# jrcalgo/RelayRL-prototype

Hardware: AMD Instinct MI355X
Metric: env steps/sec (whole node) + wall-clock to return threshold, CartPole REINFORCE (higher is better)
Workload: dtype fp32; 1 GPU; global_batch=2097152, seq_len=64, parallelism=dp1, envs_per_gpu=32768, train_vf_iters=80, hyperparams=reference defaults (gamma .98, lam .97, pi_lr 3e-4, vf_lr 1e-3)

## Files before the change

### csrc/kernels/value_grad.hip

```cpp
#include "common.h"
#include "grad_args.h"
#include "heads.h"

namespace rrl {

typedef __bf16 vbf16x8 __attribute__((ext_vector_type(8)));
typedef __bf16 vbf16x4 __attribute__((ext_vector_type(4)));
typedef short vs16x4 __attribute__((ext_vector_type(4)));

constexpr int kVgH = 128;
#ifndef VG_MT2
#define VG_MT2 1
#endif
constexpr int kVgLd = 144;
constexpr int kVgImg = 64 * kVgLd;
constexpr int vg_red_bytes(int NA) { return 8 * 64 * NA * 4; }
constexpr int vg_base_bytes(int DP, int NA) {
  return 6 * kVgImg * 2 + 2 * 64 * DP * 4 + (2 + NA) * 128 * 4 + 32 * 4 + kVgH * kVgLd * 2;
}
constexpr bool vg_red_in_image(int DP, int NA) { return vg_base_bytes(DP, NA) + vg_red_bytes(NA) > 160 * 1024; }
constexpr int vg_lds_bytes(int DP, int NA) {
  return vg_base_bytes(DP, NA) + (vg_red_in_image(DP, NA) ? 0 : vg_red_bytes(NA));
}
constexpr bool vg_factor(int DP, int HEAD, int NA) {
// ... 3 lines not shown
constexpr int vg_hbuf_bytes(int HEAD, int NA) {
  return HEAD == HEAD_VALUE_MSE ? 0 : 64 * 4 * (2 + ((HEAD == HEAD_PG_GAUSS || HEAD == HEAD_PPO_GAUSS) ? NA : 1));
}
constexpr bool vg_split_head(int HEAD, int NA) {
  return (HEAD == HEAD_PG_GAUSS || HEAD == HEAD_PPO_GAUSS) && NA > 1;
}
constexpr int vg_dtab_bytes(int HEAD, int NA) { return vg_split_head(HEAD, NA) ? (64 + 16) * NA * 4 : 0; }
constexpr int vg_dw_bytes(int DP, int HEAD, int NA) {
  return (vg_factor(DP, HEAD, NA) || (HEAD == HEAD_VALUE_MSE && vg_lds_bytes(DP, 1) + 8 * 64 * 4 <= 160 * 1024))
             ? 8 * 64 * 4
             : 0;
}
constexpr bool vg_hbuf2(int DP, int HEAD, int NA) {
  return !vg_red_in_image(DP, NA) && vg_lds_bytes(DP, NA) + vg_mask_bytes(DP, HEAD, NA) +
                                             2 * vg_hbuf_bytes(HEAD, NA) + vg_dtab_bytes(HEAD, NA) +
                                             vg_dw_bytes(DP, HEAD, NA) <=
                                         160 * 1024;
}
constexpr int vg_total_bytes(int DP, int HEAD, int NA) {
  return vg_lds_bytes(DP, NA) + vg_mask_bytes(DP, HEAD, NA) +
         (vg_red_in_image(DP, NA) ? 0 : (vg_hbuf2(DP, HEAD, NA) ? 2 : 1) * vg_hbuf_bytes(HEAD, NA)) +
         vg_dtab_bytes(HEAD, NA) + vg_dw_bytes(DP, HEAD, NA);
}
static_assert(vg_red_bytes(6) + vg_hbuf_bytes(HEAD_PPO_GAUSS, 6) <= 3 * kVgImg * 2, "head inputs in the dh2 image");
static_assert(vg_total_bytes(8, HEAD_VALUE_MSE, 1) <= 160 * 1024, "factored LDS plan");
static_assert(vg_total_bytes(4, HEAD_PG_CAT, 2) <= 160 * 1024 && vg_total_bytes(4, HEAD_PPO_CAT, 2) <= 160 * 1024,
              "factored binary policy LDS plan");
static_assert(vg_dw_bytes(20, HEAD_VALUE_MSE, 1) > 0 && vg_total_bytes(20, HEAD_VALUE_MSE, 1) <= 160 * 1024,
              "dout table of the D = 17..20 value kernel");
static_assert(vg_lds_bytes(24, 1) <= 160 * 1024 && !vg_red_in_image(24, 1), "value-grad LDS plan");
static_assert(vg_lds_bytes(20, 6) <= 160 * 1024, "value-grad LDS plan exceeds 160 KB");
static_assert(vg_red_bytes(6) <= 3 * kVgImg * 2, "head partials must fit in the dh2 image");

struct Split8 {
  vbf16x8 h, m, l;
};

struct Split8HM {
  vbf16x8 h, m;
};

typedef float vf32x2 __attribute__((ext_vector_type(2)));

RRL_DEV uint32_t cvt_pk_bf16(float a, float b) {
  typedef __bf16 vbf16x2_cvt __attribute__((ext_vector_type(2)));
  return __builtin_bit_cast(uint32_t, __builtin_convertvector((vf32x2{a, b}), vbf16x2_cvt));
// ... 163 lines not shown
  const bool hi = j & 1;
  const float send = hi ? w2[0] : w2[1], keep = hi ? w2[1] : w2[0];
  return keep + dpp_f<kDppXor1>(send);
}

RRL_DEV float wave_sum_vl(float v) {
  v += dpp_f<kDppXor1>(v);
  v += dpp_f<kDppXor2>(v);
  v += dpp_f<kDppMirror8>(v);
  v += dpp_f<kDppXor8>(v);
  return group_sum_swap(v);
}

#define VG_STAMP(k)                                                                     \
  if (STAMP) {                                                                          \
    __builtin_amdgcn_sched_barrier(0);                                                  \
    unsigned long long t_;                                                              \
    asm volatile("s_memtime %0\n\ts_waitcnt lgkmcnt(0)" : "=s"(t_)::"memory");          \
    __builtin_amdgcn_sched_barrier(0);                                                  \
    if ((k) > 0) st_sum[(k) > 0 ? (k)-1 : 0] += t_ - st_prev;                           \
    st_prev = t_;                                                                       \
  }

constexpr int vg_prod_v(int DP) { return DP <= 4 ? 3 : 1; }

template <int DP, int HEAD, int NA, bool STAMP = false, int V = vg_prod_v(DP), bool FWD = false>
__global__ __launch_bounds__(512, 1) void value_grad_split_kernel(GradArgs p) {
  unsigned long long st_prev = 0, st_sum[12] = {0, 0, 0, 0, 0, 0, 0, 0, 0, 0, 0, 0};
  unsigned long long st_entry = 0;
  if (STAMP) asm volatile("s_memtime %0\n\ts_waitcnt lgkmcnt(0)" : "=s"(st_entry)::"memory");
  extern __shared__ __attribute__((aligned(16))) uint16_t vg_lds[];
  constexpr bool kValue = HEAD == HEAD_VALUE_MSE;
  constexpr bool kGauss = HEAD == HEAD_PG_GAUSS || HEAD == HEAD_PPO_GAUSS;
  constexpr bool kPPO = HEAD == HEAD_PPO_CAT || HEAD == HEAD_PPO_GAUSS;
  static_assert(!kValue || NA == 1, "the value head has one output");
  static_assert(!FWD || kValue, "the forward-only instance is the value head's");
  static_assert(NA >= 1 && NA <= 6, "NA <= 6 (LDS plan, two field groups)");
  static_assert(!vg_split_head(HEAD, NA) || (NA % 2 == 0 && NA <= 6),
                "the dout table is read in output pairs; head MFMA lanes g = 0, 1 hold outputs 0..7");
  constexpr bool kFactor = vg_factor(DP, HEAD, NA) && !FWD;
  constexpr bool kBin = kFactor && !kValue;
  constexpr bool kMaskB = kFactor && (V & 1);
  constexpr bool kInterleave = kMaskB && (V & 2);
  constexpr int NF = NA + 2;
  constexpr int NG = (NF + 3) / 4;
  constexpr bool kRedImg = vg_red_in_image(DP, NA);
  constexpr bool kSplitHead = vg_split_head(HEAD, NA);
  uint16_t* h1img = vg_lds;
  uint16_t* dhimg = vg_lds + 3 * kVgImg;
  float* tail = reinterpret_cast<float*>(vg_lds + 6 * kVgImg);
  float* red = kRedImg ? reinterpret_cast<float*>(dhimg) : tail;
  float* xsb = kRedImg ? tail : tail + 8 * NA * 64;
  float* vecs = xsb + 2 * 64 * DP;
  uint16_t* w2lo = reinterpret_cast<uint16_t*>(vecs + (2 + NA) * kVgH + 32);
  uint32_t* mk = reinterpret_cast<uint32_t*>(w2lo + kVgH * kVgLd);
  const vbf16x8* mtab = reinterpret_cast<const vbf16x8*>(mk + 64 * 4);
  float* hbuf0 = kRedImg ? red + 8 * NA * 64
                         : reinterpret_cast<float*>(reinterpret_cast<char*>(mk) + vg_mask_bytes(DP, HEAD, NA));
  float* dtab = reinterpret_cast<float*>(
      reinterpret_cast<char*>(mk) + vg_mask_bytes(DP, HEAD, NA) +
      (kRedImg ? 0 : (vg_hbuf2(DP, HEAD, NA) ? 2 : 1) * vg_hbuf_bytes(HEAD, NA)));
  float* hacc = dtab + 64 * NA;
  if (kSplitHead && lane_id() < 2 * NA) hacc[(threadIdx.x >> 6) * 2 * NA + lane_id()] = 0.f;
  if (kMaskB) {
    for (int q = threadIdx.x; q < 256 * 4; q += blockDim.x) {
      const int i = q >> 2, e = 2 * (q & 3);
      mk[64 * 4 + q] = (((i >> e) & 1) ? 0x3F80u : 0u) | (((i >> (e + 1)) & 1) ? 0x3F800000u : 0u);
    }
  }
  int parity = 0;
  constexpr int KS1 = DP / 4;
  const int l = lane_id();
  const int j = l & 15, g = l >> 4, w = threadIdx.x >> 6;
  const int D = p.D;
  const int Bv = p.nvalid ? min(*p.nvalid, p.B) : p.B;
  const int Bc = max(Bv, 1);
  const float invB = p.inv_B_dev ? *p.inv_B_dev : p.inv_B;
  const FlatOffsets o = flat_offsets(D, kVgH, NA);
  float adv_mean = 0.f, adv_rstd = 1.f;
  if (!kValue && p.adv_stats != nullptr) {
    const float n = fmaxf(p.adv_stats[2], 1.f);
    adv_mean = p.adv_stats[0] / n;
    const float var = fmaxf(p.adv_stats[1] / n - adv_mean * adv_mean, 0.f);
    adv_rstd = 1.f / (sqrtf(var) + 1e-8f);
  }
  const float* __restrict__ P = p.params;
  const int own = 16 * w;

  constexpr int NC = kGauss ? NA : 1;
  const int wu = __builtin_amdgcn_readfirstlane(w);
  auto dma = [&](const void* src, long n, long first, float* dst, int chunks, int w0) {
    for (int k = 0; k < chunks; ++k) {
      if (((k + w0) & 7) == wu) {
        const long e = min(first + 64L * k + l, n - 1);
        __builtin_amdgcn_global_load_lds(static_cast<const uint32_t*>(src) + e,
                                         (__attribute__((address_space(3))) void*)(dst + 64 * k), 4, 0, 0);
      }
    }
  };
  constexpr bool kDmaIn = !kValue;
  constexpr int XQ = (64 * DP + 511) / 512;
  float xr[kDmaIn ? 1 : XQ];
  float hin_r = 0.f;
  auto prefetch_x = [&](int b0, float* dst) {
    if (kDmaIn) {
      for (int k = wu; k < DP; k += 8) {
        const int q = 64 * k + l, row = q / DP, d = q % DP;
        const long e = (long)min(b0 + row, Bc - 1) * D + min(d, D - 1);
        __builtin_amdgcn_global_load_lds(static_cast<const uint32_t*>(static_cast<const void*>(p.X)) + e,
                                         (__attribute__((address_space(3))) void*)(dst + 64 * k), 4, 0, 0);
      }
    } else {
#pragma unroll
      for (int i = 0; i < (kDmaIn ? 1 : XQ); ++i) {
        const int q = min((int)threadIdx.x + 512 * i, 64 * DP - 1);
        const int rl = q / DP, d = q % DP, b = b0 + rl;
        xr[i] = p.X[(size_t)min(b, Bc - 1) * D + min(d, D - 1)];
      }
      if (!FWD) hin_r = p.ret[min(b0 + l, p.B - 1)];
    }
  };
  constexpr bool kHb2 = kDmaIn && vg_hbuf2(DP, HEAD, NA);
  constexpr int HBF = vg_hbuf_bytes(HEAD, NA) / 4;
  auto dma_head = [&](int b0, float* hbuf) {
    if (kDmaIn) {
      dma(p.adv, p.B, b0, hbuf, 1, 3);
      if (p.logp_old) dma(p.logp_old, p.B, b0, hbuf + 64, 1, 4);
      if (kGauss) dma(p.actc, (long)p.B * NA, (long)b0 * NA, hbuf + 128, NA, 5);
      else dma(p.act, p.B, b0, hbuf + 128, 1, 5);
    }
  };
  auto vm_wait0 = []() { __builtin_amdgcn_s_waitcnt(0x0F70); };
  prefetch_x(blockIdx.x * 64, xsb);
  if (kHb2) dma_head(blockIdx.x * 64, hbuf0);

  constexpr int kW2Ld = kVgH + 4;
  static_assert(kVgH * kW2Ld * 4 <= 6 * kVgImg * 2, "staged W2 must fit in the activation images");
  float* w2s = reinterpret_cast<float*>(vg_lds);
  float* hsc = vecs + (2 + NA) * kVgH;
  float w1a[KS1];
#pragma unroll
  for (int s = 0; s < KS1; ++s) {
    const int k = 4 * s + g;
    w1a[s] = (k < D) ? P[o.w1 + (own + j) * D + k] : 0.f;
// ... 12 lines not shown
        for (int e = 0; e < 4; ++e) v[it][e] = gw2[4 * q + e];
      }
    }
    for (int q = threadIdx.x; q < (2 + NA) * kVgH; q += blockDim.x) {
      const int k = q >> 7, f = q & (kVgH - 1);
      vecs[q] = P[(k == 0 ? o.b1 : k == 1 ? o.b2 : o.w3 + (k - 2) * kVgH) + f];
    }
    if (threadIdx.x < NA) {
      const int a = threadIdx.x;
      const float lsa = kGauss ? P[o.log_std + a] : 0.f;
      hsc[a] = P[o.b3 + a];
      hsc[NA + a] = lsa;
      hsc[2 * NA + a] = __expf(-lsa);
    }
#pragma unroll
    for (int it = 0; it < kVgH * kVgH / 4 / 512; ++it) {
      const int q = (int)threadIdx.x + 512 * it;
      *reinterpret_cast<floatx4*>(w2s + (q >> 5) * kW2Ld + 4 * (q & 31)) = v[it];
      vbf16x4 h, m, lo;
      split4(v[it], h, m, lo);
      *reinterpret_cast<vbf16x4*>(w2lo + (q >> 5) * kVgLd + 4 * (q & 31)) = lo;
    }
  }
  __syncthreads();
  Split8HM wA[4], wB[4];
  auto w3f = [&](int k) { return kBin ? vecs[3 * kVgH + k] - vecs[2 * kVgH + k] : vecs[2 * kVgH + k]; };
  vbf16x8 wBl[kFactor ? 4 : 1];
#pragma unroll
  for (int c = 0; c < 4; ++c) {
    const floatx4 a0 = *reinterpret_cast<const floatx4*>(w2s + (own + j) * kW2Ld + 32 * c + 8 * g);
    const floatx4 a1 = *reinterpret_cast<const floatx4*>(w2s + (own + j) * kW2Ld + 32 * c + 8 * g + 4);
    const Split8 sa = split8(a0, a1);
    wA[c].h = sa.h;
    wA[c].m = sa.m;
    if constexpr (!FWD) {
      floatx4 b0, b1;
#pragma unroll
      for (int e = 0; e < 4; ++e) {
        b0[e] = w2s[(32 * c + 8 * g + e) * kW2Ld + own + j];
        b1[e] = w2s[(32 * c + 8 * g + 4 + e) * kW2Ld + own + j];
        if (kFactor) {
          b0[e] *= w3f(32 * c + 8 * g + e);
          b1[e] *= w3f(32 * c + 8 * g + 4 + e);
        }
      }
      const Split8 sb = split8(b0, b1);
      wB[c].h = sb.h;
      wB[c].m = sb.m;
      if (kFactor) wBl[c % (kFactor ? 4 : 1)] = sb.l;
    }
  }
  const float* b1p = vecs + own + 4 * g;
  const float* b2p = vecs + kVgH + own + 4 * g;
  const float* w3p = vecs + 2 * kVgH + own + 4 * g;

  floatx4 acc2[8];
  float accv[NG];
  constexpr bool kDw1Mfma = DP > 4;
  constexpr int kTail1 = (DP > 16 && DP % 16 == 4) ? 4 : 0;
  constexpr int NT1 = kTail1 ? DP / 16 : (DP + 15) / 16;
  constexpr int NA1 = kDw1Mfma ? (kTail1 ? kTail1 : 1) : DP;
  float acc1[NA1];
  floatx4 acc1m[kDw1Mfma ? NT1 : 1];
  float db1acc = 0.f;
#pragma unroll
  for (int it = 0; it < 8; ++it) acc2[it] = zero4();
#pragma unroll
  for (int q = 0; q < NG; ++q) accv[q] = 0.f;
#pragma unroll
  for (int d = 0; d < NA1; ++d) acc1[d] = 0.f;
#pragma unroll
  for (int nt = 0; nt < (kDw1Mfma ? NT1 : 1); ++nt) acc1m[nt] = zero4();
  float bacc3 = 0.f, dls = 0.f;
  constexpr bool kTvPersist = kFactor && DP == 4;
  float tvs[kFactor ? 16 : 1];
#pragma unroll
  for (int e = 0; e < (kFactor ? 16 : 1); ++e) tvs[e] = 0.f;
  auto fold_tvs = [&]() {
    float tf[16];
#pragma unroll
    for (int e = 0; e < 16; ++e) {
      constexpr int TN = kFactor ? 16 : 1;
      if (!kFactor) tf[e] = 0.f;
      else if (!kBin) tf[e] = tvs[e % TN];
      else tf[e] = e < 4 ? tvs[e % TN] : e < 8 ? -tvs[e % TN] : e < 12 ? 0.f : tvs[(e - 8) % TN];
    }
    return reduce_scatter16(tf, j);
  };
  float s_loss = 0.f, s_val = 0.f, s_cnt = 0.f, s_ent = 0.f, s_kl = 0.f, s_clip = 0.f;

  if ((p.tune & 1) && __builtin_amdgcn_readfirstlane(threadIdx.x) >= 256) __builtin_amdgcn_s_setprio(1);
  if ((p.tune & 2) && __builtin_amdgcn_readfirstlane(threadIdx.x) < 256) __builtin_amdgcn_s_setprio(1);

  VG_STAMP(0);
  if (STAMP) st_sum[10] = st_prev - st_entry;
  for (int base = blockIdx.x * 64; base < Bv; base += gridDim.x * 64) {
    VG_STAMP(0);
    float* xs = xsb + (parity & 1) * 64 * DP;
    float* hbuf = hbuf0 + (kHb2 ? (parity & 1) * HBF : 0);
    parity ^= 1;
    if (kDmaIn) {
      vm_wait0();
    } else {
#pragma unroll
      for (int i = 0; i < (kDmaIn ? 1 : XQ); ++i) {
        const int q = (int)threadIdx.x + 512 * i;
        const int rl = q / DP, d = q % DP;
        if (q < 64 * DP) xs[q] = (base + rl < Bv && d < D) ? xr[i] : 0.f;
      }
    }
    __syncthreads();
    VG_STAMP(1);

    {
      float xv[4][KS1];
#pragma unroll
      for (int bt = 0; bt < 4; ++bt) {
#pragma unroll
        for (int s = 0; s < KS1; ++s) xv[bt][s] = xs[(16 * bt + j) * DP + 4 * s + g];
      }
      const floatx4 b1v = *reinterpret_cast<const floatx4*>(b1p);
      floatx4 a1[4];
#pragma unroll
      for (int bt = 0; bt < 4; ++bt) {
        a1[bt] = b1v;
#pragma unroll
        for (int s = 0; s < KS1; ++s) a1[bt] = mfma4(w1a[s], xv[bt][s], a1[bt]);
      }
#pragma unroll
      for (int bt = 0; bt < 4; ++bt) {
#pragma unroll
        for (int r = 0; r < 4; ++r) a1[bt][r] = relu1(a1[bt][r]);
        store_split(h1img, 16 * bt + j, own + 4 * g, a1[bt]);
      }
    }
    __syncthreads();
    if (kDmaIn && !kHb2) dma_head(base, hbuf);

    VG_STAMP(2);
    floatx4 h2[4];
#pragma unroll
    for (int bt = 0; bt < 4; ++bt) h2[bt] = *reinterpret_cast<const floatx4*>(b2p);
    {
      Split8 cur = frag_row(h1img, j, 8 * g);
      vbf16x8 al = *reinterpret_cast<const vbf16x8*>(w2lo + (own + j) * kVgLd + 8 * g);
#pragma unroll
      for (int it = 0; it < 16; ++it) {
        const int c = it >> 2, bt = it & 3;
        Split8 nxt;
        vbf16x8 aln;
        if (it + 1 < 16) nxt = frag_row(h1img, 16 * ((it + 1) & 3) + j, 32 * ((it + 1) >> 2) + 8 * g);
        if (bt == 3 && it + 1 < 16)
          aln = *reinterpret_cast<const vbf16x8*>(w2lo + (own + j) * kVgLd + 32 * (c + 1) + 8 * g);
        const Split8 a{wA[c].h, wA[c].m, al};
        h2[bt] = mma6(a, cur, h2[bt]);
        __builtin_amdgcn_sched_barrier(0);
        if (it + 1 < 16) cur = nxt;
        if (bt == 3 && it + 1 < 16) al = aln;
      }
    }
#pragma unroll
    for (int bt = 0; bt < 4; ++bt) {
#pragma unroll
      for (int r = 0; r < 4; ++r) h2[bt][r] = relu1(h2[bt][r]);
    }
    if (kMaskB) {
      uint32_t x01 = 0, x23 = 0;
#pragma unroll
      for (int bt = 0; bt < 4; ++bt) {
        uint32_t nib = 0;
#pragma unroll
        for (int r = 0; r < 4; ++r) nib |= (h2[bt][r] > 0.f ? 1u : 0u) << r;
        const uint32_t sh = 4 * g + 16 * (bt & 1);
        if (bt < 2) x01 |= nib << sh;
        else x23 |= nib << sh;
      }
      x01 = group_or_swap(x01);
      x23 = group_or_swap(x23);
      const uint32_t u = ((g < 2 ? x01 : x23) >> (16 * (g & 1))) & 0xffffu;
      uint8_t* mb = reinterpret_cast<uint8_t*>(mk) + (16 * g + j) * 16 + 8 * (w & 1) + (w >> 1);
      mb[0] = (uint8_t)(u & 0xffu);
      mb[4] = (uint8_t)(u >> 8);
    }

    VG_STAMP(3);
    if constexpr (kSplitHead) {
      floatx4 w3m = zero4();
      if (j < NA) w3m = *reinterpret_cast<const floatx4*>(w3p + j * kVgH);
#pragma unroll
      for (int bt = 0; bt < 4; ++bt) {
        floatx4 c = zero4();
#pragma unroll
        for (int r = 0; r < 4; ++r) c = mfma4(w3m[r], h2[bt][r], c);
        float* dst = red + (w * 64 + 16 * bt + j) * NA + 4 * g;
        if (g == 0) {
          *reinterpret_cast<vf32x2*>(dst) = vf32x2{c[0], c[1]};
          *reinterpret_cast<vf32x2*>(dst + 2) = vf32x2{c[2], c[3]};
        } else if (4 * g < NA) {
          *reinterpret_cast<vf32x2*>(dst) = vf32x2{c[0], c[1]};
        }
      }
    } else {
#pragma unroll
    for (int a = 0; a < NA; ++a) {
      const floatx4 w3a = *reinterpret_cast<const floatx4*>(w3p + a * kVgH);
// ... 161 lines not shown
          s_cnt += 1.f;
        }
      }
      float mb = 0.f, ml = 0.f;
#pragma unroll
      for (int a = 0; a < NA; ++a) {
        if (a == w) {
          mb = dout[a];
          if (kGauss) ml = dls_row[a % NC];
        }
      }
      if (w < NA) {
        bacc3 += wave_sum_vl(mb);
        if (kGauss) dls += wave_sum_vl(ml);
      }
    }
    auto prefetch_next = [&]() {
      if (base + (int)gridDim.x * 64 < Bv) {
        prefetch_x(base + gridDim.x * 64, xsb + (parity & 1) * 64 * DP);
        if (kHb2) dma_head(base + gridDim.x * 64, hbuf0 + (parity & 1) * HBF);
      }
    };
    constexpr bool kHeadBar = kRedImg || kSplitHead;
    if (!kHeadBar && kFactor) prefetch_next();
    if (kHeadBar) {
      __syncthreads();
      prefetch_next();
    }

    VG_STAMP(6);
    floatx4 dh1[4];
#pragma unroll
    for (int bt = 0; bt < 4; ++bt) dh1[bt] = zero4();
    auto dh1_relu = [&]() {
#pragma unroll
      for (int cc = 0; cc < 2; ++cc) {
        typedef unsigned short vu16x8 __attribute__((ext_vector_type(8)));
        const vu16x8 hb = __builtin_bit_cast(vu16x8, frag_tr1(h1img, 32 * cc, own, l));
#pragma unroll
        for (int e = 0; e < 8; ++e) {
          const int bt = 2 * cc + (e >> 2), i = e & 3;
          dh1[bt][i] = hb[e] != 0 ? dh1[bt][i] : 0.f;
          db1acc += dh1[bt][i];
        }
      }
    };
    constexpr bool kDwTab = vg_dw_bytes(DP, HEAD, NA) > 0 && (kMaskB || !kFactor);
    float* dtw = reinterpret_cast<float*>(reinterpret_cast<char*>(vg_lds) + vg_total_bytes(DP, HEAD, NA) -
                                          vg_dw_bytes(DP, HEAD, NA)) + 64 * w;
    if (kFactor) {
      const float dfac = kBin ? 0.5f * (dout[NA - 1] - dout[0]) : dout[0];
      float dv[4];
      if (kMaskB) {
        dtw[l] = dfac;
        __builtin_amdgcn_fence(__ATOMIC_ACQ_REL, "wavefront");
        __builtin_amdgcn_wave_barrier();
#pragma unroll
        for (int bt = 0; bt < 4; ++bt) dv[bt] = dtw[16 * bt + j];
      } else {
#pragma unroll
        for (int bt = 0; bt < 4; ++bt) dv[bt] = __shfl(dfac, 16 * bt + j, 64);
      }
      float* tv = tvs;
      if (!kTvPersist) {
#pragma unroll
        for (int e = 0; e < 16; ++e) tvs[e % (kFactor ? 16 : 1)] = 0.f;
      }
      auto kf_tile = [&](const int bt) {
        const float v = dv[bt];
        uint32_t ph, pm, pl;
        split2(vf32x2{v, v}, ph, pm, pl);
        uint32_t mw[2];
#pragma unroll
        for (int q = 0; q < 2; ++q) {
          const bool p0 = h2[bt][2 * q] > 0.f, p1 = h2[bt][2 * q + 1] > 0.f;
          mw[q] = (p0 ? 0x0000ffffu : 0u) | (p1 ? 0xffff0000u : 0u);
        }
        Pieces pc;
        pc.h = __builtin_bit_cast(vbf16x4, make_uint2(mw[0] & ph, mw[1] & ph));
        pc.m = __builtin_bit_cast(vbf16x4, make_uint2(mw[0] & pm, mw[1] & pm));
        pc.l = __builtin_bit_cast(vbf16x4, make_uint2(mw[0] & pl, mw[1] & pl));
        store_pieces(dhimg, 16 * bt + j, own + 4 * g, pc);
#pragma unroll
        for (int r = 0; r < 4; ++r) {
          tv[r] += h2[bt][r] > 0.f ? v : 0.f;
          tv[4 + r] = fmaf(v, h2[bt][r], tv[4 + r]);
        }
      };
      auto kf_finish = [&]() {
        if (!kTvPersist) accv[0] += fold_tvs();
        if (kMaskB) {
          __builtin_amdgcn_fence(__ATOMIC_ACQ_REL, "wavefront");
          __builtin_amdgcn_wave_barrier();
        }
      };
      auto kf_dh2 = [&]() {
#pragma unroll
        for (int bt = 0; bt < 4; ++bt) kf_tile(bt);
        kf_finish();
      };
      auto kf_dh1 = [&]() {
        if (kMaskB) {
          uint32_t mrow[4];
#pragma unroll
          for (int bt = 0; bt < 4; ++bt) mrow[bt] = mk[(16 * bt + j) * 4 + g];
          constexpr int kAhead = VG_MT2 ? 2 : 1;
          auto mfrag = [&](int it) { return mtab[(mrow[it & 3] >> (8 * (it >> 2))) & 0xffu]; };
          vbf16x8 q0 = mfrag(0), q1;
          if (kAhead == 2) q1 = mfrag(1);
#pragma unroll
          for (int it = 0; it < 16; ++it) {
            const int c = it >> 2, bt = it & 3;
            vbf16x8 nxt;
            if (it + kAhead < 16) nxt = mfrag(it + kAhead);
            dh1[bt] = mfma_bf16(q0, wBl[c % (kFactor ? 4 : 1)], dh1[bt]);
            dh1[bt] = mfma_bf16(q0, wB[c].m, dh1[bt]);
            dh1[bt] = mfma_bf16(q0, wB[c].h, dh1[bt]);
            if (kInterleave) {
              if ((it & 3) == 1) kf_tile(it >> 2);
              if (it == 15) kf_finish();
            }
            __builtin_amdgcn_sched_barrier(0);
            if (kAhead == 2) {
              q0 = q1;
              if (it + 2 < 16) q1 = nxt;
            } else if (it + 1 < 16) {
              q0 = nxt;
            }
          }
        } else {
          vbf16x8 cur = *reinterpret_cast<const vbf16x8*>(dhimg + img_off(j, 8 * g));
#pragma unroll
          for (int it = 0; it < 16; ++it) {
            const int c = it >> 2, bt = it & 3;
            vbf16x8 nxt;
            if (it + 1 < 16)
              nxt = *reinterpret_cast<const vbf16x8*>(
                  dhimg + img_off(16 * ((it + 1) & 3) + j, 32 * ((it + 1) >> 2) + 8 * g));
            dh1[bt] = mfma_bf16(cur, wBl[c % (kFactor ? 4 : 1)], dh1[bt]);
            dh1[bt] = mfma_bf16(cur, wB[c].m, dh1[bt]);
            dh1[bt] = mfma_bf16(cur, wB[c].h, dh1[bt]);
            __builtin_amdgcn_sched_barrier(0);
            if (it + 1 < 16) cur = nxt;
          }
// ... 164 lines not shown
            floatx4 x[DP / 4];
            load_xrow(16 * bt + 4 * g + i, x);
            dw1_rows_valu(bt, i, x);
          }
        }
      }
    };
    auto do_dw2 = [&]() {
      VG_STAMP(9);
      Split8 a = frag_tr(dhimg, 0, own, l);
      Split8 cur = frag_tr(h1img, 0, 0, l);
#pragma unroll
      for (int it = 0; it < 16; ++it) {
        const int t = it & 7;
        Split8 nxt, an;
        if (it + 1 < 16) nxt = frag_tr(h1img, 32 * ((it + 1) >> 3), 16 * ((it + 1) & 7), l);
        if (it == 7) an = frag_tr(dhimg, 32, own, l);
        acc2[t] = mma6(a, cur, acc2[t]);
        __builtin_amdgcn_sched_barrier(0);
        if (it + 1 < 16) cur = nxt;
        if (it == 7) a = an;
      }
    };
    auto do_dw2_dw1 = [&]() {
      VG_STAMP(8);
      VG_STAMP(9);
      Split8 a = frag_tr(dhimg, 0, own, l);
      Split8 cur = frag_tr(h1img, 0, 0, l);
      floatx4 xq[DP / 4];
      load_xrow(4 * g, xq);
#pragma unroll
      for (int it = 0; it < 16; ++it) {
        const int t = it & 7;
        Split8 nxt, an;
        if (it + 1 < 16) nxt = frag_tr(h1img, 32 * ((it + 1) >> 3), 16 * ((it + 1) & 7), l);
        if (it == 7) an = frag_tr(dhimg, 32, own, l);
        acc2[t] = mma6(a, cur, acc2[t]);
        {
          floatx4 xc[DP / 4];
#pragma unroll
          for (int d4 = 0; d4 < DP / 4; ++d4) xc[d4] = xq[d4];
          if (it + 1 < 16) load_xrow(16 * ((it + 1) >> 2) + 4 * g + ((it + 1) & 3), xq);
          dw1_rows_valu(it >> 2, it & 3, xc);
        }
        __builtin_amdgcn_sched_barrier(0);
        if (it + 1 < 16) cur = nxt;
        if (it == 7) a = an;
      }
    };
    if (kInterleave && !kDw1Mfma) {
      do_dw2_dw1();
    } else {
      do_dw1();
      do_dw2();
    }
    VG_STAMP(10);
  }

  if constexpr (FWD) return;
  if (kTvPersist) accv[0] += fold_tvs();
  float* slab = p.grad_slab + (size_t)blockIdx.x * p.P;
  auto w3g = [&](int f) { return kBin ? P[o.w3 + kVgH + f] - P[o.w3 + f] : P[o.w3 + f]; };
  floatx4 w3s;
#pragma unroll
  for (int r = 0; r < 4; ++r) w3s[r] = kFactor ? w3g(own + 4 * g + r) : 1.f;
#pragma unroll
  for (int it = 0; it < 8; ++it) {
#pragma unroll
    for (int r = 0; r < 4; ++r) slab[o.w2 + (own + 4 * g + r) * kVgH + 16 * it + j] = acc2[it][r] * w3s[r];
  }
#pragma unroll
  for (int q = 0; q < NG; ++q) {
    const int f = 4 * q + (j >> 2), feat = own + 4 * g + (j & 3);
    if (f < NF) {
      const int off = f == 0 ? o.b2 : f == 1 ? o.w3 : f == 2 ? o.b1 : o.w3 + (f == 3 ? 1 : f - 2) * kVgH;
      if (f != 2) slab[off + feat] = (kFactor && f == 0) ? accv[q] * w3g(feat) : accv[q];
    }
  }
  if (kDw1Mfma) {
#pragma unroll
    for (int nt = 0; nt < (kDw1Mfma ? NT1 : 1); ++nt) {
#pragma unroll
      for (int i = 0; i < 4; ++i) {
        const int d = 16 * nt + j;
        if (d < D) slab[o.w1 + (own + 4 * g + i) * D + d] = acc1m[nt][i];
      }
    }
#pragma unroll
    for (int e = 0; e < kTail1; ++e) {
      const float sd = group_sum_swap(acc1[e % NA1]);
      const int d = 16 * NT1 + e;
      if (g == e && d < D) slab[o.w1 + (own + j) * D + d] = sd;
    }
  } else {
#pragma unroll
    for (int d = 0; d < NA1; ++d) {
      const float sd = group_sum_swap(acc1[d]);
      if (g == (d & 3) && d < D) slab[o.w1 + (own + j) * D + d] = sd;
    }
  }
  {
    const float sb = group_sum_swap(db1acc);
    if (g == 0) slab[o.b1 + own + j] = sb;
  }
  if constexpr (kSplitHead) {
    const float st[6] = {wave_sum_vl(s_loss), wave_sum_vl(s_ent), wave_sum_vl(s_kl),
                         wave_sum_vl(s_clip), wave_sum_vl(s_val), wave_sum_vl(s_cnt)};
    __syncthreads();
    float* ep = dtab;
    if (l == 0) {
#pragma unroll
      for (int k = 0; k < 6; ++k) ep[w * 6 + k] = st[k];
    }
    __syncthreads();
    const int t = threadIdx.x;
    if (t < 2 * NA) {
      float v = 0.f;
#pragma unroll
      for (int ww = 0; ww < 8; ++ww) v += hacc[ww * 2 * NA + t];
      slab[(t < NA ? o.b3 : o.log_std - NA) + t] = v;
    } else if (t >= 64 && t < 70) {
      float v = 0.f;
#pragma unroll
      for (int ww = 0; ww < 8; ++ww) v += ep[ww * 6 + t - 64];
      p.loss_slab[blockIdx.x * 8 + t - 64] = v;
    }
  }
  if (!kSplitHead && w < NA && l == 0) {
    slab[o.b3 + w] = bacc3;
    if (kGauss) slab[o.log_std + w] = dls;
  }
  if (!kSplitHead && w == 0) {
    const float sl = wave_sum(s_loss), sv = wave_sum(s_val), sc = wave_sum(s_cnt);
    const float se = wave_sum(s_ent), sk = wave_sum(s_kl), scl = wave_sum(s_clip);
    if (l == 0) {
      float* lsl = p.loss_slab + blockIdx.x * 8;
      lsl[0] = sl;
      lsl[1] = se;
      lsl[2] = sk;
      lsl[3] = scl;
      lsl[4] = sv;
      lsl[5] = sc;
    }
  }
  if (STAMP && p.stamps != nullptr) {
    unsigned long long t_end;
    asm volatile("s_memtime %0\n\ts_waitcnt lgkmcnt(0)" : "=s"(t_end)::"memory");
    st_sum[11] = t_end - st_prev;
    if (l == 0) {
#pragma unroll
      for (int k = 0; k < 12; ++k) p.stamps[(blockIdx.x * 8 + w) * 16 + k] = st_sum[k];
    }
  }
}

bool value_grad_split_supported(int D, int H) { return H == kVgH && D >= 1 && D <= 24; }

bool policy_grad_split_supported(int D, int H, int A, int head) {
  if (H != kVgH || D < 1) return false;
  if (head == HEAD_PG_CAT || head == HEAD_PPO_CAT) return D <= 8 && A >= 2 && A <= 4;
  if (head == HEAD_PG_GAUSS || head == HEAD_PPO_GAUSS) return D <= 20 && (A == 1 || A == 6);
  return false;
}

static int g_vg_tune = 0;
static unsigned long long* g_vg_stamps = nullptr;

template <int DP, int HEAD, int NA, bool STAMP, int V>
static int launch_inst(const GradArgs& a, int grid, hipStream_t s) {
  constexpr int bytes = vg_total_bytes(DP, HEAD, NA);
  static_assert(bytes <= 160 * 1024, "value-grad LDS plan exceeds 160 KB");
  static bool attr_set = false;
  if (!attr_set) {
    (void)hipFuncSetAttribute((const void*)value_grad_split_kernel<DP, HEAD, NA, STAMP, V>,
                              hipFuncAttributeMaxDynamicSharedMemorySize, bytes);
    attr_set = true;
  }
  hipLaunchKernelGGL((value_grad_split_kernel<DP, HEAD, NA, STAMP, V>), dim3(grid), dim3(512), bytes, s, a);
  return (int)hipGetLastError();
}

template <int DP, int HEAD, int NA, bool STAMP>
static int launch_var(const GradArgs& a, int grid, hipStream_t s) {
  if constexpr (HEAD == HEAD_VALUE_MSE && DP <= 8) {
    if (a.tune & 128) {
      switch ((a.tune >> 4) & 7) {
        case 0: return launch_inst<DP, HEAD, NA, STAMP, 0>(a, grid, s);
        case 1: return launch_inst<DP, HEAD, NA, STAMP, 1>(a, grid, s);
        case 3: return launch_inst<DP, HEAD, NA, STAMP, 3>(a, grid, s);
        default: break;
      }
    }
  }
  return launch_inst<DP, HEAD, NA, STAMP, vg_prod_v(DP)>(a, grid, s);
}

template <int DP, int HEAD, int NA>
static int launch_vg(const GradArgs& a0, int grid, hipStream_t s) {
  GradArgs a = a0;
  a.tune = g_vg_tune;
  a.stamps = g_vg_stamps;
  if (a.tune & 8) return launch_var<DP, HEAD, NA, true>(a, grid, s);
  return launch_var<DP, HEAD, NA, false>(a, grid, s);
}

int launch_value_grad_split(const GradArgs& a, int grid, hipStream_t s) {
  if (a.D <= 4) return launch_vg<4, HEAD_VALUE_MSE, 1>(a, grid, s);
  if (a.D <= 8) return launch_vg<8, HEAD_VALUE_MSE, 1>(a, grid, s);
  if (a.D <= 16) return launch_vg<16, HEAD_VALUE_MSE, 1>(a, grid, s);
  if (a.D <= 20) return launch_vg<20, HEAD_VALUE_MSE, 1>(a, grid, s);
  return launch_vg<24, HEAD_VALUE_MSE, 1>(a, grid, s);
}

template <int DP>
static int launch_fwd(const GradArgs& a0, int grid, hipStream_t s) {
// ... 75 lines not shown
```

Before: 33.23 million env_steps/s.

## Software-pipeline layer-1 forward of next batch into layer-2 MFMA loop for D<=4 value grad

Adds a pipelined variant (V=7) of the value-gradient kernel for D<=4 that computes the next tile's layer-1 activations into a double-buffered h1 image while the current tile's layer-2 MFMAs run. X gets a triple buffer so it can be loaded two tiles ahead. The dW2 A-operand is rebuilt from a compact relu-mask table plus a split dout table instead of writing and re-reading the dh image. This removes a barrier and a serial layer-1 phase per tile, at the cost of extra LDS, tighter hand-written scheduling barriers and higher register pressure. It becomes the default for DP=4, with a fallback to the old variant when each block handles only one tile.

```diff
diff --git a/csrc/kernels/value_grad.hip b/csrc/kernels/value_grad.hip
--- a/csrc/kernels/value_grad.hip
+++ b/csrc/kernels/value_grad.hip
@@ -1,3 +1,5 @@
+#include <type_traits>
+
 #include "common.h"
 #include "grad_args.h"
 #include "heads.h"
@@ -49,6 +51,13 @@
          (vg_red_in_image(DP, NA) ? 0 : (vg_hbuf2(DP, HEAD, NA) ? 2 : 1) * vg_hbuf_bytes(HEAD, NA)) +
          vg_dtab_bytes(HEAD, NA) + vg_dw_bytes(DP, HEAD, NA);
 }
+constexpr bool vg_pipe(int DP, int HEAD, int V) { return HEAD == HEAD_VALUE_MSE && DP == 4 && (V & 7) == 7; }
+constexpr int vg_pipe_bytes(int DP, int HEAD, int V) {
+  return vg_pipe(DP, HEAD, V) ? 64 * DP * 4 + 8 * 64 * 2 + 3 * 64 * 2 : 0;
+}
+static_assert(vg_total_bytes(4, HEAD_VALUE_MSE, 1) % 16 == 0 &&
+                  vg_total_bytes(4, HEAD_VALUE_MSE, 1) + vg_pipe_bytes(4, HEAD_VALUE_MSE, 7) <= 160 * 1024,
+              "pipelined layer-1 LDS plan");
 static_assert(vg_red_bytes(6) + vg_hbuf_bytes(HEAD_PPO_GAUSS, 6) <= 3 * kVgImg * 2, "head inputs in the dh2 image");
 static_assert(vg_total_bytes(8, HEAD_VALUE_MSE, 1) <= 160 * 1024, "factored LDS plan");
 static_assert(vg_total_bytes(4, HEAD_PG_CAT, 2) <= 160 * 1024 && vg_total_bytes(4, HEAD_PPO_CAT, 2) <= 160 * 1024,
@@ -258,7 +267,7 @@
     st_prev = t_;                                                                       \
   }
 
-constexpr int vg_prod_v(int DP) { return DP <= 4 ? 3 : 1; }
+constexpr int vg_prod_v(int DP) { return DP <= 4 ? 7 : 1; }
 
 template <int DP, int HEAD, int NA, bool STAMP = false, int V = vg_prod_v(DP), bool FWD = false>
 __global__ __launch_bounds__(512, 1) void value_grad_split_kernel(GradArgs p) {
@@ -278,6 +287,7 @@
   constexpr bool kBin = kFactor && !kValue;
   constexpr bool kMaskB = kFactor && (V & 1);
   constexpr bool kInterleave = kMaskB && (V & 2);
+  constexpr bool kPipe = kInterleave && !FWD && vg_pipe(DP, HEAD, V);
   constexpr int NF = NA + 2;
   constexpr int NG = (NF + 3) / 4;
   constexpr bool kRedImg = vg_red_in_image(DP, NA);
@@ -297,6 +307,9 @@
       reinterpret_cast<char*>(mk) + vg_mask_bytes(DP, HEAD, NA) +
       (kRedImg ? 0 : (vg_hbuf2(DP, HEAD, NA) ? 2 : 1) * vg_hbuf_bytes(HEAD, NA)));
   float* hacc = dtab + 64 * NA;
+  float* xs3 = reinterpret_cast<float*>(reinterpret_cast<char*>(vg_lds) + vg_total_bytes(DP, HEAD, NA));
+  uint16_t* mbt = reinterpret_cast<uint16_t*>(xs3 + 64 * DP) + 64 * (threadIdx.x >> 6);
+  uint16_t* dpt = reinterpret_cast<uint16_t*>(xs3 + 64 * DP) + 8 * 64;
   if (kSplitHead && lane_id() < 2 * NA) hacc[(threadIdx.x >> 6) * 2 * NA + lane_id()] = 0.f;
   if (kMaskB) {
     for (int q = threadIdx.x; q < 256 * 4; q += blockDim.x) {
@@ -305,6 +318,7 @@
     }
   }
   int parity = 0;
+  int xi = 0;
   constexpr int KS1 = DP / 4;
   const int l = lane_id();
   const int j = l & 15, g = l >> 4, w = threadIdx.x >> 6;
@@ -322,6 +336,11 @@
   }
   const float* __restrict__ P = p.params;
   const int own = 16 * w;
+  auto frag_slot = [&]() {
+    int ll = l;
+    asm volatile("" : "+v"(ll));
+    return (ll & 32) + 8 * ((ll >> 2) & 3) + ((ll >> 2) & 4) + (ll & 3);
+  };
 
   constexpr int NC = kGauss ? NA : 1;
   const int wu = __builtin_amdgcn_readfirstlane(w);
@@ -356,6 +375,27 @@
       if (!FWD) hin_r = p.ret[min(b0 + l, p.B - 1)];
     }
   };
+  auto xbuf = [&](int i) { return i < 2 ? xsb + i * 64 * DP : xs3; };
+  auto load_x = [&](int b0) {
+    int tid = threadIdx.x;
+    asm volatile("" : "+v"(tid));
+#pragma unroll
+    for (int i = 0; i < (kDmaIn ? 1 : XQ); ++i) {
+      const int q = min(tid + 512 * i, 64 * DP - 1);
+      const int rl = q / DP, d = q % DP, b = b0 + rl;
+      xr[i] = p.X[(size_t)min(b, Bc - 1) * D + min(d, D - 1)];
+    }
+  };
+  auto store_x = [&](int b0, float* dst) {
+    int tid = threadIdx.x;
+    asm volatile("" : "+v"(tid));
+#pragma unroll
+    for (int i = 0; i < (kDmaIn ? 1 : XQ); ++i) {
+      const int q = tid + 512 * i;
+      const int rl = q / DP, d = q % DP;
+      if (q < 64 * DP) dst[q] = (b0 + rl < Bv && d < D) ? xr[i] : 0.f;
+    }
+  };
   constexpr bool kHb2 = kDmaIn && vg_hbuf2(DP, HEAD, NA);
   constexpr int HBF = vg_hbuf_bytes(HEAD, NA) / 4;
   auto dma_head = [&](int b0, float* hbuf) {
@@ -414,6 +454,10 @@
       *reinterpret_cast<vbf16x4*>(w2lo + (q >> 5) * kVgLd + 4 * (q & 31)) = lo;
     }
   }
+  if constexpr (kPipe) {
+    store_x(blockIdx.x * 64, xsb);
+    if ((int)(blockIdx.x + gridDim.x) * 64 < Bv) load_x((blockIdx.x + gridDim.x) * 64);
+  }
   __syncthreads();
   Split8HM wA[4], wB[4];
   auto w3f = [&](int k) { return kBin ? vecs[3 * kVgH + k] - vecs[2 * kVgH + k] : vecs[2 * kVgH + k]; };
@@ -445,6 +489,33 @@
   const float* b1p = vecs + own + 4 * g;
   const float* b2p = vecs + kVgH + own + 4 * g;
   const float* w3p = vecs + 2 * kVgH + own + 4 * g;
+
+  auto layer1 = [&](const float* xs, uint16_t* img) {
+    float xv[4][KS1];
+#pragma unroll
+    for (int bt = 0; bt < 4; ++bt) {
+#pragma unroll
+      for (int s = 0; s < KS1; ++s) xv[bt][s] = xs[(16 * bt + j) * DP + 4 * s + g];
+    }
+    const floatx4 b1v = *reinterpret_cast<const floatx4*>(b1p);
+    floatx4 a1[4];
+#pragma unroll
+    for (int bt = 0; bt < 4; ++bt) {
+      a1[bt] = b1v;
+#pragma unroll
+      for (int s = 0; s < KS1; ++s) a1[bt] = mfma4(w1a[s], xv[bt][s], a1[bt]);
+    }
+#pragma unroll
+    for (int bt = 0; bt < 4; ++bt) {
+#pragma unroll
+      for (int r = 0; r < 4; ++r) a1[bt][r] = relu1(a1[bt][r]);
+      store_split(img, 16 * bt + j, own + 4 * g, a1[bt]);
+    }
+  };
+  if constexpr (kPipe) {
+    __syncthreads();
+    layer1(xsb, vg_lds);
+  }
 
   floatx4 acc2[8];
   float accv[NG];
@@ -488,10 +559,17 @@
   if (STAMP) st_sum[10] = st_prev - st_entry;
   for (int base = blockIdx.x * 64; base < Bv; base += gridDim.x * 64) {
     VG_STAMP(0);
-    float* xs = xsb + (parity & 1) * 64 * DP;
+    float* xs = kPipe ? xbuf(xi) : xsb + (parity & 1) * 64 * DP;
     float* hbuf = hbuf0 + (kHb2 ? (parity & 1) * HBF : 0);
+    uint16_t* const h1s = kPipe ? vg_lds + (parity & 1) * 3 * kVgImg : h1img;
+    uint16_t* const h1n = vg_lds + ((parity & 1) ^ 1) * 3 * kVgImg;
+    const int xin = xi == 2 ? 0 : xi + 1;
+    const float* xsn = xbuf(xin);
+    xi = xin;
     parity ^= 1;
-    if (kDmaIn) {
+    if constexpr (kPipe) {
+      store_x(base + (int)gridDim.x * 64, xbuf(xin));
+    } else if (kDmaIn) {
       vm_wait0();
     } else {
 #pragma unroll
@@ -504,36 +582,78 @@
     __syncthreads();
     VG_STAMP(1);
 
-    {
-      float xv[4][KS1];
-#pragma unroll
-      for (int bt = 0; bt < 4; ++bt) {
-#pragma unroll
-        for (int s = 0; s < KS1; ++s) xv[bt][s] = xs[(16 * bt + j) * DP + 4 * s + g];
-      }
-      const floatx4 b1v = *reinterpret_cast<const floatx4*>(b1p);
-      floatx4 a1[4];
-#pragma unroll
-      for (int bt = 0; bt < 4; ++bt) {
-        a1[bt] = b1v;
-#pragma unroll
-        for (int s = 0; s < KS1; ++s) a1[bt] = mfma4(w1a[s], xv[bt][s], a1[bt]);
-      }
-#pragma unroll
-      for (int bt = 0; bt < 4; ++bt) {
-#pragma unroll
-        for (int r = 0; r < 4; ++r) a1[bt][r] = relu1(a1[bt][r]);
-        store_split(h1img, 16 * bt + j, own + 4 * g, a1[bt]);
-      }
-    }
-    __syncthreads();
+    if constexpr (!kPipe) {
+      layer1(xs, h1img);
+      __syncthreads();
+    }
     if (kDmaIn && !kHb2) dma_head(base, hbuf);
 
     VG_STAMP(2);
     floatx4 h2[4];
 #pragma unroll
     for (int bt = 0; bt < 4; ++bt) h2[bt] = *reinterpret_cast<const floatx4*>(b2p);
-    {
+    if constexpr (kPipe) {
+      auto fwd_steps = [&](auto look) {
+        constexpr bool kLook = decltype(look)::value;
+        int tf = threadIdx.x;
+        asm volatile("" : "+v"(tf));
+        const int jl = tf & 15, gl = (tf >> 4) & 3, ownl = 16 * (tf >> 6);
+        const float* b1l = vecs + ownl + 4 * gl;
+        Split8 cur = frag_row(h1s, j, 8 * g);
+        vbf16x8 al = *reinterpret_cast<const vbf16x8*>(w2lo + (own + j) * kVgLd + 8 * g);
+        float xv;
+        floatx4 t1;
+        uint32_t ph[2], pm[2], pl[2];
+        auto store_tile = [&](int t) {
+          Pieces pc;
+          pc.h = __builtin_bit_cast(vbf16x4, make_uint2(ph[0], ph[1]));
+          pc.m = __builtin_bit_cast(vbf16x4, make_uint2(pm[0], pm[1]));
+          pc.l = __builtin_bit_cast(vbf16x4, make_uint2(pl[0], pl[1]));
+          store_pieces(h1n, 16 * t + jl, ownl + 4 * gl, pc);
+        };
+#pragma unroll
+        for (int it = 0; it < 16; ++it) {
+          const int c = it >> 2, bt = it & 3;
+          Split8 nxt;
+          vbf16x8 aln;
+          if (it + 1 < 16) nxt = frag_row(h1s, 16 * ((it + 1) & 3) + j, 32 * ((it + 1) >> 2) + 8 * g);
+          if (bt == 3 && it + 1 < 16)
+            aln = *reinterpret_cast<const vbf16x8*>(w2lo + (own + j) * kVgLd + 32 * (c + 1) + 8 * g);
+          const int lt = it >> 2, ls = it & 3;
+          if (kLook && ls == 0) {
+            xv = xsn[(16 * lt + jl) * DP + gl];
+            t1 = *reinterpret_cast<const floatx4*>(b1l);
+          }
+          if (kLook && ls == 1) t1 = mfma4(w1a[0], xv, t1);
+          const Split8 a{wA[c].h, wA[c].m, al};
+          h2[bt] = mma6(a, cur, h2[bt]);
+          if (kLook && ls >= 2) {
+            const int q = ls - 2;
+            split2(vf32x2{relu1(t1[2 * q]), relu1(t1[2 * q + 1])}, ph[q], pm[q], pl[q]);
+          }
+          if (kLook && ls == 3) store_tile(lt);
+          if (it == 0) __builtin_amdgcn_sched_group_barrier(0x100, 10, 0);
+          else if (ls == 0) __builtin_amdgcn_sched_group_barrier(0x100, kLook ? 5 : 3, 0);
+          else if (ls == 3) {
+            __builtin_amdgcn_sched_group_barrier(0x002, 3, 0);
+            __builtin_amdgcn_sched_group_barrier(0x100, 4, 0);
+          } else {
+            __builtin_amdgcn_sched_group_barrier(0x100, 3, 0);
+          }
+          if (kLook && ls == 1) __builtin_amdgcn_sched_group_barrier(0x008, 1, 0);
+#pragma unroll
+          for (int k = 0; k < 6; ++k) {
+            __builtin_amdgcn_sched_group_barrier(0x008, 1, 0);
+            __builtin_amdgcn_sched_group_barrier(0x002, 3, 0);
+          }
+          __builtin_amdgcn_sched_barrier(0);
+          if (it + 1 < 16) cur = nxt;
+          if (bt == 3 && it + 1 < 16) al = aln;
+        }
+      };
+      if (base + (int)gridDim.x * 64 < Bv) fwd_steps(std::true_type{});
+      else fwd_steps(std::false_type{});
+    } else {
       Split8 cur = frag_row(h1img, j, 8 * g);
       vbf16x8 al = *reinterpret_cast<const vbf16x8*>(w2lo + (own + j) * kVgLd + 8 * g);
 #pragma unroll
@@ -573,6 +693,7 @@
       uint8_t* mb = reinterpret_cast<uint8_t*>(mk) + (16 * g + j) * 16 + 8 * (w & 1) + (w >> 1);
       mb[0] = (uint8_t)(u & 0xffu);
       mb[4] = (uint8_t)(u >> 8);
+      if constexpr (kPipe) mbt[frag_slot()] = (uint16_t)u;
     }
 
     VG_STAMP(3);
@@ -780,7 +901,15 @@
       }
     };
     constexpr bool kHeadBar = kRedImg || kSplitHead;
-    if (!kHeadBar && kFactor) prefetch_next();
+    if constexpr (kPipe) {
+      const int stride = (int)gridDim.x * 64;
+      if (base + stride < Bv) {
+        hin_r = p.ret[min(base + stride + l, p.B - 1)];
+        if (base + 2 * stride < Bv) load_x(base + 2 * stride);
+      }
+    } else if (!kHeadBar && kFactor) {
+      prefetch_next();
+    }
     if (kHeadBar) {
       __syncthreads();
       prefetch_next();
@@ -794,7 +923,7 @@
 #pragma unroll
       for (int cc = 0; cc < 2; ++cc) {
         typedef unsigned short vu16x8 __attribute__((ext_vector_type(8)));
-        const vu16x8 hb = __builtin_bit_cast(vu16x8, frag_tr1(h1img, 32 * cc, own, l));
+        const vu16x8 hb = __builtin_bit_cast(vu16x8, frag_tr1(h1s, 32 * cc, own, l));
 #pragma unroll
         for (int e = 0; e < 8; ++e) {
           const int bt = 2 * cc + (e >> 2), i = e & 3;
@@ -826,19 +955,21 @@
       }
       auto kf_tile = [&](const int bt) {
         const float v = dv[bt];
-        uint32_t ph, pm, pl;
-        split2(vf32x2{v, v}, ph, pm, pl);
-        uint32_t mw[2];
-#pragma unroll
-        for (int q = 0; q < 2; ++q) {
-          const bool p0 = h2[bt][2 * q] > 0.f, p1 = h2[bt][2 * q + 1] > 0.f;
-          mw[q] = (p0 ? 0x0000ffffu : 0u) | (p1 ? 0xffff0000u : 0u);
-        }
-        Pieces pc;
-        pc.h = __builtin_bit_cast(vbf16x4, make_uint2(mw[0] & ph, mw[1] & ph));
-        pc.m = __builtin_bit_cast(vbf16x4, make_uint2(mw[0] & pm, mw[1] & pm));
-        pc.l = __builtin_bit_cast(vbf16x4, make_uint2(mw[0] & pl, mw[1] & pl));
-        store_pieces(dhimg, 16 * bt + j, own + 4 * g, pc);
+        if constexpr (!kPipe) {
+          uint32_t ph, pm, pl;
+          split2(vf32x2{v, v}, ph, pm, pl);
+          uint32_t mw[2];
+#pragma unroll
+          for (int q = 0; q < 2; ++q) {
+            const bool p0 = h2[bt][2 * q] > 0.f, p1 = h2[bt][2 * q + 1] > 0.f;
+            mw[q] = (p0 ? 0x0000ffffu : 0u) | (p1 ? 0xffff0000u : 0u);
+          }
+          Pieces pc;
+          pc.h = __builtin_bit_cast(vbf16x4, make_uint2(mw[0] & ph, mw[1] & ph));
+          pc.m = __builtin_bit_cast(vbf16x4, make_uint2(mw[0] & pm, mw[1] & pm));
+          pc.l = __builtin_bit_cast(vbf16x4, make_uint2(mw[0] & pl, mw[1] & pl));
+          store_pieces(dhimg, 16 * bt + j, own + 4 * g, pc);
+        }
 #pragma unroll
         for (int r = 0; r < 4; ++r) {
           tv[r] += h2[bt][r] > 0.f ? v : 0.f;
@@ -874,10 +1005,21 @@
             dh1[bt] = mfma_bf16(q0, wBl[c % (kFactor ? 4 : 1)], dh1[bt]);
             dh1[bt] = mfma_bf16(q0, wB[c].m, dh1[bt]);
             dh1[bt] = mfma_bf16(q0, wB[c].h, dh1[bt]);
+            if constexpr (kPipe) {
+              if (it == 0) {
+                uint32_t ph, pm, pl;
+                split2(vf32x2{dfac, dfac}, ph, pm, pl);
+                uint16_t* dp = dpt + frag_slot();
+                dp[0] = (uint16_t)ph;
+                dp[64] = (uint16_t)pm;
+                dp[128] = (uint16_t)pl;
+              }
+            }
             if (kInterleave) {
               if ((it & 3) == 1) kf_tile(it >> 2);
               if (it == 15) kf_finish();
             }
+            if constexpr (kPipe) __builtin_amdgcn_sched_group_barrier(0x100, 1, 0);
             __builtin_amdgcn_sched_barrier(0);
             if (kAhead == 2) {
               q0 = q1;
@@ -1088,19 +1230,42 @@
         if (it == 7) a = an;
       }
     };
+    auto a_frag = [&](int c) {
+      typedef uint32_t vu32x4 __attribute__((ext_vector_type(4)));
+      const vu32x4 mb = *reinterpret_cast<const vu32x4*>(mbt + 32 * c + 8 * g);
+      const uint16_t* tp = dpt + 32 * c + 8 * g;
+      vu32x4 m;
+#pragma unroll
+      for (int k = 0; k < 4; ++k) {
+        const uint32_t lo = (uint32_t)__builtin_amdgcn_sbfe((int)mb[k], (uint32_t)j, 1u);
+        const uint32_t hi = (uint32_t)__builtin_amdgcn_sbfe((int)mb[k], (uint32_t)(j + 16), 1u);
+        m[k] = (lo & 0x0000ffffu) | (hi & 0xffff0000u);
+      }
+      Split8 a;
+      a.h = __builtin_bit_cast(vbf16x8, m & *reinterpret_cast<const vu32x4*>(tp));
+      a.m = __builtin_bit_cast(vbf16x8, m & *reinterpret_cast<const vu32x4*>(tp + 64));
+      a.l = __builtin_bit_cast(vbf16x8, m & *reinterpret_cast<const vu32x4*>(tp + 128));
+      return a;
+    };
     auto do_dw2_dw1 = [&]() {
       VG_STAMP(8);
       VG_STAMP(9);
-      Split8 a = frag_tr(dhimg, 0, own, l);
-      Split8 cur = frag_tr(h1img, 0, 0, l);
+      Split8 a;
+      if constexpr (kPipe) a = a_frag(0);
+      else a = frag_tr(dhimg, 0, own, l);
+      Split8 cur = frag_tr(h1s, 0, 0, l);
       floatx4 xq[DP / 4];
       load_xrow(4 * g, xq);
 #pragma unroll
       for (int it = 0; it < 16; ++it) {
         const int t = it & 7;
         Split8 nxt, an;
-        if (it + 1 < 16) nxt = frag_tr(h1img, 32 * ((it + 1) >> 3), 16 * ((it + 1) & 7), l);
-        if (it == 7) an = frag_tr(dhimg, 32, own, l);
+        if (it + 1 < 16) nxt = frag_tr(h1s, 32 * ((it + 1) >> 3), 16 * ((it + 1) & 7), l);
+        if constexpr (kPipe) {
+          if (it == 7) an = a_frag(1);
+        } else {
+          if (it == 7) an = frag_tr(dhimg, 32, own, l);
+        }
         acc2[t] = mma6(a, cur, acc2[t]);
         {
           floatx4 xc[DP / 4];
@@ -1125,97 +1290,102 @@
 
   if constexpr (FWD) return;
   if (kTvPersist) accv[0] += fold_tvs();
-  float* slab = p.grad_slab + (size_t)blockIdx.x * p.P;
-  auto w3g = [&](int f) { return kBin ? P[o.w3 + kVgH + f] - P[o.w3 + f] : P[o.w3 + f]; };
-  floatx4 w3s;
-#pragma unroll
-  for (int r = 0; r < 4; ++r) w3s[r] = kFactor ? w3g(own + 4 * g + r) : 1.f;
-#pragma unroll
-  for (int it = 0; it < 8; ++it) {
-#pragma unroll
-    for (int r = 0; r < 4; ++r) slab[o.w2 + (own + 4 * g + r) * kVgH + 16 * it + j] = acc2[it][r] * w3s[r];
-  }
-#pragma unroll
-  for (int q = 0; q < NG; ++q) {
-    const int f = 4 * q + (j >> 2), feat = own + 4 * g + (j & 3);
-    if (f < NF) {
-      const int off = f == 0 ? o.b2 : f == 1 ? o.w3 : f == 2 ? o.b1 : o.w3 + (f == 3 ? 1 : f - 2) * kVgH;
-      if (f != 2) slab[off + feat] = (kFactor && f == 0) ? accv[q] * w3g(feat) : accv[q];
-    }
-  }
-  if (kDw1Mfma) {
-#pragma unroll
-    for (int nt = 0; nt < (kDw1Mfma ? NT1 : 1); ++nt) {
-#pragma unroll
-      for (int i = 0; i < 4; ++i) {
-        const int d = 16 * nt + j;
-        if (d < D) slab[o.w1 + (own + 4 * g + i) * D + d] = acc1m[nt][i];
-      }
-    }
-#pragma unroll
-    for (int e = 0; e < kTail1; ++e) {
-      const float sd = group_sum_swap(acc1[e % NA1]);
-      const int d = 16 * NT1 + e;
-      if (g == e && d < D) slab[o.w1 + (own + j) * D + d] = sd;
-    }
-  } else {
-#pragma unroll
-    for (int d = 0; d < NA1; ++d) {
-      const float sd = group_sum_swap(acc1[d]);
-      if (g == (d & 3) && d < D) slab[o.w1 + (own + j) * D + d] = sd;
-    }
-  }
+  int te = threadIdx.x;
+  if constexpr (kPipe) asm volatile("" : "+v"(te));
   {
-    const float sb = group_sum_swap(db1acc);
-    if (g == 0) slab[o.b1 + own + j] = sb;
-  }
-  if constexpr (kSplitHead) {
-    const float st[6] = {wave_sum_vl(s_loss), wave_sum_vl(s_ent), wave_sum_vl(s_kl),
-                         wave_sum_vl(s_clip), wave_sum_vl(s_val), wave_sum_vl(s_cnt)};
-    __syncthreads();
-    float* ep = dtab;
-    if (l == 0) {
-#pragma unroll
-      for (int k = 0; k < 6; ++k) ep[w * 6 + k] = st[k];
-    }
-    __syncthreads();
-    const int t = threadIdx.x;
-    if (t < 2 * NA) {
-      float v = 0.f;
-#pragma unroll
-      for (int ww = 0; ww < 8; ++ww) v += hacc[ww * 2 * NA + t];
-      slab[(t < NA ? o.b3 : o.log_std - NA) + t] = v;
-    } else if (t >= 64 && t < 70) {
-      float v = 0.f;
-#pragma unroll
-      for (int ww = 0; ww < 8; ++ww) v += ep[ww * 6 + t - 64];
-      p.loss_slab[blockIdx.x * 8 + t - 64] = v;
-    }
-  }
-  if (!kSplitHead && w < NA && l == 0) {
-    slab[o.b3 + w] = bacc3;
-    if (kGauss) slab[o.log_std + w] = dls;
-  }
-  if (!kSplitHead && w == 0) {
-    const float sl = wave_sum(s_loss), sv = wave_sum(s_val), sc = wave_sum(s_cnt);
-    const float se = wave_sum(s_ent), sk = wave_sum(s_kl), scl = wave_sum(s_clip);
-    if (l == 0) {
-      float* lsl = p.loss_slab + blockIdx.x * 8;
-      lsl[0] = sl;
-      lsl[1] = se;
-      lsl[2] = sk;
-      lsl[3] = scl;
-      lsl[4] = sv;
-      lsl[5] = sc;
-    }
-  }
-  if (STAMP && p.stamps != nullptr) {
-    unsigned long long t_end;
-    asm volatile("s_memtime %0\n\ts_waitcnt lgkmcnt(0)" : "=s"(t_end)::"memory");
-    st_sum[11] = t_end - st_prev;
-    if (l == 0) {
-#pragma unroll
-      for (int k = 0; k < 12; ++k) p.stamps[(blockIdx.x * 8 + w) * 16 + k] = st_sum[k];
+    const int l = te & 63, j = l & 15, g = l >> 4, w = te >> 6, own = 16 * w;
+    float* slab = p.grad_slab + (size_t)blockIdx.x * p.P;
+    auto w3g = [&](int f) { return kBin ? P[o.w3 + kVgH + f] - P[o.w3 + f] : P[o.w3 + f]; };
+    floatx4 w3s;
+#pragma unroll
+    for (int r = 0; r < 4; ++r) w3s[r] = kFactor ? w3g(own + 4 * g + r) : 1.f;
+#pragma unroll
+    for (int it = 0; it < 8; ++it) {
+#pragma unroll
+      for (int r = 0; r < 4; ++r) slab[o.w2 + (own + 4 * g + r) * kVgH + 16 * it + j] = acc2[it][r] * w3s[r];
+    }
+#pragma unroll
+    for (int q = 0; q < NG; ++q) {
+      const int f = 4 * q + (j >> 2), feat = own + 4 * g + (j & 3);
+      if (f < NF) {
+        const int off = f == 0 ? o.b2 : f == 1 ? o.w3 : f == 2 ? o.b1 : o.w3 + (f == 3 ? 1 : f - 2) * kVgH;
+        if (f != 2) slab[off + feat] = (kFactor && f == 0) ? accv[q] * w3g(feat) : accv[q];
+      }
+    }
+    if (kDw1Mfma) {
+#pragma unroll
+      for (int nt = 0; nt < (kDw1Mfma ? NT1 : 1); ++nt) {
+#pragma unroll
+        for (int i = 0; i < 4; ++i) {
+          const int d = 16 * nt + j;
+          if (d < D) slab[o.w1 + (own + 4 * g + i) * D + d] = acc1m[nt][i];
+        }
+      }
+#pragma unroll
+      for (int e = 0; e < kTail1; ++e) {
+        const float sd = group_sum_swap(acc1[e % NA1]);
+        const int d = 16 * NT1 + e;
+        if (g == e && d < D) slab[o.w1 + (own + j) * D + d] = sd;
+      }
+    } else {
+#pragma unroll
+      for (int d = 0; d < NA1; ++d) {
+        const float sd = group_sum_swap(acc1[d]);
+        if (g == (d & 3) && d < D) slab[o.w1 + (own + j) * D + d] = sd;
+      }
+    }
+    {
+      const float sb = group_sum_swap(db1acc);
+      if (g == 0) slab[o.b1 + own + j] = sb;
+    }
+    if constexpr (kSplitHead) {
+      const float st[6] = {wave_sum_vl(s_loss), wave_sum_vl(s_ent), wave_sum_vl(s_kl),
+                           wave_sum_vl(s_clip), wave_sum_vl(s_val), wave_sum_vl(s_cnt)};
+      __syncthreads();
+      float* ep = dtab;
+      if (l == 0) {
+#pragma unroll
+        for (int k = 0; k < 6; ++k) ep[w * 6 + k] = st[k];
+      }
+      __syncthreads();
+      const int t = threadIdx.x;
+      if (t < 2 * NA) {
+        float v = 0.f;
+#pragma unroll
+        for (int ww = 0; ww < 8; ++ww) v += hacc[ww * 2 * NA + t];
+        slab[(t < NA ? o.b3 : o.log_std - NA) + t] = v;
+      } else if (t >= 64 && t < 70) {
+        float v = 0.f;
+#pragma unroll
+        for (int ww = 0; ww < 8; ++ww) v += ep[ww * 6 + t - 64];
+        p.loss_slab[blockIdx.x * 8 + t - 64] = v;
+      }
+    }
+    if (!kSplitHead && w < NA && l == 0) {
+      slab[o.b3 + w] = bacc3;
+      if (kGauss) slab[o.log_std + w] = dls;
+    }
+    if (!kSplitHead && w == 0) {
+      const float sl = wave_sum(s_loss), sv = wave_sum(s_val), sc = wave_sum(s_cnt);
+      const float se = wave_sum(s_ent), sk = wave_sum(s_kl), scl = wave_sum(s_clip);
+      if (l == 0) {
+        float* lsl = p.loss_slab + blockIdx.x * 8;
+        lsl[0] = sl;
+        lsl[1] = se;
+        lsl[2] = sk;
+        lsl[3] = scl;
+        lsl[4] = sv;
+        lsl[5] = sc;
+      }
+    }
+    if (STAMP && p.stamps != nullptr) {
+      unsigned long long t_end;
+      asm volatile("s_memtime %0\n\ts_waitcnt lgkmcnt(0)" : "=s"(t_end)::"memory");
+      st_sum[11] = t_end - st_prev;
+      if (l == 0) {
+#pragma unroll
+        for (int k = 0; k < 12; ++k) p.stamps[(blockIdx.x * 8 + w) * 16 + k] = st_sum[k];
+      }
     }
   }
 }
@@ -1234,7 +1404,7 @@
 
 template <int DP, int HEAD, int NA, bool STAMP, int V>
 static int launch_inst(const GradArgs& a, int grid, hipStream_t s) {
-  constexpr int bytes = vg_total_bytes(DP, HEAD, NA);
+  constexpr int bytes = vg_total_bytes(DP, HEAD, NA) + vg_pipe_bytes(DP, HEAD, V);
   static_assert(bytes <= 160 * 1024, "value-grad LDS plan exceeds 160 KB");
   static bool attr_set = false;
   if (!attr_set) {
@@ -1254,9 +1424,15 @@
         case 0: return launch_inst<DP, HEAD, NA, STAMP, 0>(a, grid, s);
         case 1: return launch_inst<DP, HEAD, NA, STAMP, 1>(a, grid, s);
         case 3: return launch_inst<DP, HEAD, NA, STAMP, 3>(a, grid, s);
+        case 7:
+          if constexpr (DP == 4) return launch_inst<DP, HEAD, NA, STAMP, 7>(a, grid, s);
+          break;
         default: break;
       }
     }
+  }
+  if constexpr (vg_pipe(DP, HEAD, vg_prod_v(DP))) {
+    if ((long)a.B <= 64L * grid) return launch_inst<DP, HEAD, NA, STAMP, 3>(a, grid, s);
   }
   return launch_inst<DP, HEAD, NA, STAMP, vg_prod_v(DP)>(a, grid, s);
 }
```

Result: faster. 33.92 million env_steps/s, median of 6 (+2.1%).
